# LuletterSoul/RP-Style-Transfer

Hardware: AMD Instinct MI355X
Metric: stylized images/sec at 512×512, 1/2/4/8 MI355X; % HBM roofline (higher is better)
Workload: dtype fp32

## Files before the change

rp-style-transfer_amd/csrc/rpst_wino4q.hip:

```cpp
#include "rpst_conv.h"

#include <type_traits>

#ifndef RPST_W4Q_DBG
#define RPST_W4Q_DBG 0
#endif

namespace rpst {
namespace {

template <int PAD>
__device__ __forceinline__ void q_mfma(floatx4& acc, float a, float b) {
  if constexpr (PAD)
    asm volatile("s_nop 1\n\tv_mfma_f32_16x16x4_f32 %0, %1, %2, %0" : "+v"(acc) : "v"(a), "v"(b));
  else
    asm volatile("v_mfma_f32_16x16x4_f32 %0, %1, %2, %0" : "+v"(acc) : "v"(a), "v"(b));
}
__device__ __forceinline__ unsigned q_lds_addr(const float* p) {
  return (unsigned)(uintptr_t)(const __attribute__((address_space(3))) float*)p;
}
template <int OFF>
__device__ __forceinline__ void q_dma16(__amdgpu_buffer_rsrc_t r, unsigned m0, unsigned voff,
                                        int soff) {
  asm volatile("s_mov_b32 m0, %0\n\ts_nop 0\n\tbuffer_load_dwordx4 %1, %2, %3 offen offset:%4 lds"
               :: "s"(m0), "v"(voff), "s"(r), "s"(soff), "i"(OFF) : "memory");
}
__device__ __forceinline__ void q_dma4(__amdgpu_buffer_rsrc_t r, unsigned m0, unsigned voff,
                                       int soff) {
  asm volatile("s_mov_b32 m0, %0\n\ts_nop 0\n\tbuffer_load_dword %1, %2, %3 offen lds"
               :: "s"(m0), "v"(voff), "s"(r), "s"(soff) : "memory");
}
__device__ __forceinline__ void q_lds_barrier() {
  asm volatile("s_waitcnt lgkmcnt(0)" ::: "memory");
  __builtin_amdgcn_s_barrier();
}

template <int H>
__device__ __forceinline__ void q_bt3(float d0, float d1, float d2, float d3, float d4, float d5,
                                      float& u0, float& u1, float& u2) {
  if constexpr (H == 0) {
    const float A = fmaf(-4.f, d2, d4), B = fmaf(-4.f, d1, d3);
    u0 = fmaf(4.f, d0, fmaf(-5.f, d2, d4));
    u1 = A + B;
    u2 = A - B;
  } else {
    const float C = d4 - d2, E = d3 - d1;
    u0 = fmaf(2.f, E, C);
    u1 = fmaf(-2.f, E, C);
    u2 = fmaf(4.f, d1, fmaf(-5.f, d3, d5));
  }
}

}

constexpr int kQCo = 64;
constexpr int kQTH = 8, kQTW = 64;
constexpr int kQXO = 4;
constexpr int kQPS = 72;
constexpr int kQCS = 768;
constexpr int kQWS = 9216;
constexpr int kQPAT = 4 * kQCS;
constexpr int kQNTH = 512;
constexpr int kQMaxCo = 512;
constexpr int kQWPI = 5;
constexpr int kQWide = 2, kQSlow = 6;
constexpr int kQDMA4 = 3, kQDMA = 12;
constexpr int kQRP = kQPS / 4;
constexpr int kQXS = 4 * 3 * 3 * 64 * 2;
constexpr int kQWG0 = 0;
constexpr int kQPG = 5;
constexpr int kQAhead = 3;
static_assert(10 * kQRP <= kQDMA4 * 64 && kQDMA4 * 256 <= kQCS, "16-B pieces in a channel");
static_assert(10 * kQPS <= kQDMA * 64 && kQDMA * 64 <= kQCS, "4-B pieces in a channel");
static_assert(2 * kQWide >= kQDMA4 && 2 * kQSlow >= kQDMA && 8 * kQWPI >= 36, "coverage");
static_assert(2 * kQXS <= kQWS, "the exchange fits a weight stage");
static_assert((2 * kQWS + 4 * kQPAT) * 4 + 1024 + kQSlow * kQNTH * 4 + 9 * kQMaxCo * 4 <= 163840,
              "LDS");

template <typename TW>
__global__ void wino4q_pack_kernel(const TW* __restrict__ w, float* __restrict__ pk, int Cout,
                                   int Cin, int K4, int64_t per, int64_t total, int64_t sco,
                                   int64_t sci, int64_t stap) {
  int64_t t = (int64_t)blockIdx.x * blockDim.x + threadIdx.x;
  if (t >= total) return;
  const int64_t img = t / per;
  pk += img * per;
  w += img * (int64_t)Cout * Cin * 9;
  t -= img * per;
  const int cb = (int)(t & 3);
  int64_t r = t >> 2;
  const int l = (int)(r & 63);
  r >>= 6;
  const int p = (int)(r % 9);
  r /= 9;
  const int q = (int)(r & 3);
  r >>= 2;
  const int ks = (int)(r % K4);
  const int ct = (int)(r / K4);
  const int i = 3 * (q >> 1) + p / 3, jj = 3 * (q & 1) + p % 3;
  const int co = ct * kQCo + cb * 16 + (l & 15);
  const int ci = ks * 4 + (l >> 4);
  float v = 0.f;
  if (co < Cout && ci < Cin) {
    const double G[6][3] = {{0.25, 0, 0},
                            {-1.0 / 6, -1.0 / 6, -1.0 / 6},
                            {-1.0 / 6, 1.0 / 6, -1.0 / 6},
                            {1.0 / 24, 1.0 / 12, 1.0 / 6},
                            {1.0 / 24, -1.0 / 12, 1.0 / 6},
                            {0, 0, 1}};
    const TW* g = w + co * sco + ci * sci;
    double acc = 0.0;
#pragma unroll
    for (int u = 0; u < 3; ++u)
#pragma unroll
      for (int s = 0; s < 3; ++s) acc += G[i][u] * (double)g[(u * 3 + s) * stap] * G[jj][s];
    v = (float)acc;
  }
  pk[t] = v;
}

size_t wino4q_packed_floats(int Cout, int Cin) {
  return (size_t)((Cout + kQCo - 1) / kQCo) * ((Cin + 3) / 4) * kQWS;
}

int wino4q_pack(const float* w, float* pk, int Cout, int Cin, hipStream_t st) {
  const int64_t t = (int64_t)wino4q_packed_floats(Cout, Cin);
  wino4q_pack_kernel<float><<<(unsigned)((t + 255) / 256), 256, 0, st>>>(
      w, pk, Cout, Cin, (Cin + 3) / 4, t, t, (int64_t)Cin * 9, 9, 1);
  return launch_status("wino4q_pack_kernel");
}

int wino4q_pack_mix(const double* wm, float* pk, int N, int Cout, int Cin, hipStream_t st) {
  const int64_t per = (int64_t)wino4q_packed_floats(Cout, Cin), tot = (int64_t)N * per;
  wino4q_pack_kernel<double><<<(unsigned)((tot + 255) / 256), 256, 0, st>>>(
      wm, pk, Cout, Cin, (Cin + 3) / 4, per, tot, Cin, 1, (int64_t)Cout * Cin);
  return launch_status("wino4q_pack_kernel(mix)");
}

__global__ void wino4q_fold_w_kernel(const float4* __restrict__ pk, float4* __restrict__ out,
                                     const float* __restrict__ aux, int N, int Cin, int K4,
                                     int64_t per4) {
  const int64_t t = (int64_t)blockIdx.x * blockDim.x + threadIdx.x;
  if (t >= (int64_t)N * per4) return;
  const int n = (int)(t / per4);
  const int64_t u = t - (int64_t)n * per4;
  const int l = (int)(u & 63);
  const int ks = (int)((u / (kQWS / 4)) % K4);
  const int ci = ks * 4 + (l >> 4);
  const int64_t nc = (int64_t)N * Cin, i = (int64_t)n * Cin + (ci < Cin ? ci : 0);
  const float sc = ci < Cin ? aux[3 * nc + i] / aux[2 * nc + i] : 0.f;
  const float4 v = pk[u];
  out[t] = make_float4(v.x * sc, v.y * sc, v.z * sc, v.w * sc);
}

int wino4q_fold_w(const float* pk, float* out, const float* aux, int N, int Cout, int Cin,
                  hipStream_t st) {
  const int64_t per4 = (int64_t)wino4q_packed_floats(Cout, Cin) / 4, n4 = (int64_t)N * per4;
  wino4q_fold_w_kernel<<<(unsigned)((n4 + 255) / 256), 256, 0, st>>>(
      reinterpret_cast<const float4*>(pk), reinterpret_cast<float4*>(out), aux, N, Cin,
      (Cin + 3) / 4, per4);
  return launch_status("wino4q_fold_w_kernel");
}

bool wino4q_applies(int Cin, int Cout, int in_op, const ConvMode& m) {
  const int min_cin = m.quarter == 2 ? 16 : 128;
  return m.quarter && m.precise != 2 && (in_op == RPST_IN_NONE || in_op == RPST_IN_UPSAMPLE2) &&
         Cout >= 64 && Cout <= kQMaxCo &&
         Cin >= min_cin && Cin % 16 == 0;
}

ConvTiling wino4q_tiling(ConvArgs& a) {
  a.Cout_pad = (a.Cout + kQCo - 1) / kQCo * kQCo;
  a.nchunks = (a.Cin + 3) / 4;
  a.tiles_x = (a.W + kQTW - 1) / kQTW;
  a.tiles_y = (a.H + kQTH - 1) / kQTH;
  a.co_tiles = a.Cout_pad / kQCo;
  a.stat_P = a.tiles_x * a.tiles_y * 2;
  a.cosplit = 1;
  return {(int64_t)a.tiles_x * a.tiles_y * a.N, kQNTH, 4, kQTH / 4, kQTW, true};
}

struct QEpi {
  int W, H, Cout, gy0, gx0, rows, n, sidx;
  bool vec, full, bst, edge, store, pool;
  float inv, slope;
  unsigned voff[4];
  float* out;
  float* oimg;
  unsigned obytes;
  const float* btab;
  float2* statp;
  int statP;
};

__device__ __forceinline__ QEpi q_epi_ctx(int wr, int tn) {
  const KArgs L = late_args();
  QEpi e;
  e.W = L->W;
  e.H = L->H;
  e.Cout = L->Cout;
  e.slope = L->relu == RPST_ACT_RELU ? 0.f : (L->relu == RPST_ACT_LRELU ? 0.2f : 1.f);
  int btx, bty;
  w4_tile((int)blockIdx.x / L->cosplit, L->tiles_x, L->tiles_y, btx, bty, e.n);
  const int bx0 = btx * kQTW;
  e.gy0 = bty * kQTH + 4 * wr;
  e.gx0 = bx0 + 4 * tn;
  e.vec = (e.W & 3) == 0 && e.gx0 + 3 < e.W;
  e.rows = max(0, min(4, e.H - e.gy0));
  const int cols = max(0, min(kQTW, e.W - bx0));
  e.inv = e.rows * cols > 0 ? __builtin_amdgcn_rcpf((float)(e.rows * cols)) : 0.f;
  e.full = e.rows == 4 && bx0 + kQTW <= e.W;
  e.edge = e.gy0 == 0 || e.gy0 + 4 >= e.H || bx0 == 0 || bx0 + kQTW >= e.W;
  e.out = L->out;
  const int64_t plane = (int64_t)e.H * e.W;
  e.pool = L->pool_out != 0;
  e.bst = !e.pool && (e.W & 3) == 0 && (int64_t)e.Cout * plane * 4 < (1LL << 31);
  e.oimg = e.out + (int64_t)e.n * e.Cout * plane;
  const bool keep = L->skip_from <= 0 || e.n < L->skip_from;
  e.obytes = keep ? (unsigned)(e.Cout * plane * 4) : 0u;
  e.store = keep;
#pragma unroll
  for (int yy = 0; yy < 4; ++yy)
    e.voff[yy] = (yy < e.rows && e.gx0 < e.W) ? (unsigned)(((e.gy0 + yy) * e.W + e.gx0) * 4)
                                             : 0x80000000u;
  e.btab = L->btab;
  e.statp = L->stat_part;
  e.statP = L->stat_P;
  e.sidx = (bty * L->tiles_x + btx) * 2 + wr;
  return e;
}

template <bool STATS, bool BTAB, bool RELU>
__device__ __forceinline__ void q_finish(const QEpi& e, int co, float (&Y)[16], int tn) {
  const int gy0 = e.gy0, gx0 = e.gx0, rows = e.rows, n = e.n;
  const bool cok = co < e.Cout;
  if constexpr (BTAB) {
    if (e.edge) {
      const float* bt = e.btab + (cok ? co : 0) * 9;
      float b9[9];
#pragma unroll
      for (int i = 0; i < 9; ++i) b9[i] = cok ? bt[i] : 0.f;
      const float b4 = b9[4];
#pragma unroll
      for (int i = 0; i < 9; ++i) b9[i] -= b4;
#pragma unroll
      for (int yy = 0; yy < 4; ++yy) {
        const int gy = gy0 + yy;
        const int rc = gy == 0 ? 0 : (gy >= e.H - 1 ? 2 : 1);
        const float l = rc == 0 ? b9[0] : (rc == 2 ? b9[6] : b9[3]);
        const float m = rc == 0 ? b9[1] : (rc == 2 ? b9[7] : b9[4]);
        const float r = rc == 0 ? b9[2] : (rc == 2 ? b9[8] : b9[5]);
#pragma unroll
        for (int xx = 0; xx < 4; ++xx) {
          const int gx = gx0 + xx;
          Y[yy * 4 + xx] += gx == 0 ? l : (gx >= e.W - 1 ? r : m);
        }
      }
    }
  }
#pragma unroll
  for (int i = 0; i < 16; ++i)
    Y[i] = __builtin_amdgcn_fmed3f(Y[i], RELU ? 0.f : e.slope * Y[i], __builtin_inff());
  float sum = 0.f;
  if constexpr (STATS) {
    if (e.full) {
#pragma unroll
      for (int i = 0; i < 16; ++i) sum += Y[i];
    } else {
#pragma unroll
      for (int yy = 0; yy < 4; ++yy)
#pragma unroll
        for (int xx = 0; xx < 4; ++xx) sum += (yy < rows && gx0 + xx < e.W) ? Y[yy * 4 + xx] : 0.f;
    }
  }
  if ((RPST_W4Q_DBG & 64) && e.statP > -7) {
  } else if (e.bst) {
    const auto ro = rsrc_or_zero(e.oimg, e.obytes, true);
    const unsigned cofs = cok ? (unsigned)co * (unsigned)(e.H * e.W) * 4u : 0x7fffffffu;
#pragma unroll
    for (int yy = 0; yy < 4; ++yy) {
      const floatx4 v = {Y[yy * 4], Y[yy * 4 + 1], Y[yy * 4 + 2], Y[yy * 4 + 3]};
      __builtin_amdgcn_raw_buffer_store_b128(__builtin_bit_cast(u32x4, v), ro,
                                             (int)(e.voff[yy] + cofs), 0, 0);
    }
  } else if (e.pool) {
    if (cok && e.store) {
      const int Ho = (e.H + 1) >> 1, Wo = (e.W + 1) >> 1;
      float* o = e.out + (((int64_t)n * e.Cout + co) * Ho + (gy0 >> 1)) * Wo + (gx0 >> 1);
#pragma unroll
      for (int py = 0; py < 2; ++py) {
        if (2 * py >= rows) continue;
        const bool y1 = 2 * py + 1 < rows;
        float pv[2];
#pragma unroll
        for (int px = 0; px < 2; ++px) {
          const bool x1 = gx0 + 2 * px + 1 < e.W;
          const float* t = Y + (2 * py) * 4 + 2 * px;
          float v = t[0];
          if (x1) v = fmaxf(v, t[1]);
          if (y1) v = fmaxf(v, t[4]);
          if (x1 && y1) v = fmaxf(v, t[5]);
          pv[px] = v;
        }
        if (gx0 + 3 < e.W && (Wo & 1) == 0) {
          *reinterpret_cast<float2*>(o + py * Wo) = make_float2(pv[0], pv[1]);
        } else {
          if (gx0 < e.W) o[py * Wo] = pv[0];
          if (gx0 + 2 < e.W) o[py * Wo + 1] = pv[1];
        }
      }
    }
  } else if (cok && e.store) {
    float* o = e.out + (((int64_t)n * e.Cout + co) * e.H + gy0) * e.W + gx0;
#pragma unroll
    for (int yy = 0; yy < 4; ++yy) {
      if (yy < rows) {
        if (e.vec) {
          *reinterpret_cast<float4*>(o + yy * e.W) =
              make_float4(Y[yy * 4], Y[yy * 4 + 1], Y[yy * 4 + 2], Y[yy * 4 + 3]);
        } else {
#pragma unroll
          for (int xx = 0; xx < 4; ++xx)
            if (gx0 + xx < e.W) o[yy * e.W + xx] = Y[yy * 4 + xx];
        }
      }
    }
  }
  if constexpr (STATS) {
    sum = row16_sum(sum);
    const float mean = sum * e.inv;
    float m2 = 0.f;
    if (e.full) {
#pragma unroll
      for (int i = 0; i < 16; ++i) m2 = fmaf(Y[i] - mean, Y[i] - mean, m2);
    } else {
#pragma unroll
      for (int yy = 0; yy < 4; ++yy)
#pragma unroll
        for (int xx = 0; xx < 4; ++xx) {
          const float dv = Y[yy * 4 + xx] - mean;
          m2 += (yy < rows && gx0 + xx < e.W) ? dv * dv : 0.f;
        }
    }
    m2 = row16_sum(m2);
    if (tn == 0 && cok)
      e.statp[((int64_t)n * e.statP + e.sidx) * e.Cout + co] = make_float2(mean, m2);
  }
}

template <int INOP, bool STATS, bool BTAB, bool RELU>
__global__ __launch_bounds__(kQNTH, 1) void wino4q_mfma_kernel(ConvArgs a) {
  __shared__ __attribute__((aligned(16))) float ws0[kQWS];
  __shared__ __attribute__((aligned(16))) float ws1[kQWS];
  __shared__ __attribute__((aligned(16))) float ps0[kQPAT];
  __shared__ __attribute__((aligned(16))) float ps1[kQPAT];
  __shared__ __attribute__((aligned(16))) float ps2[kQPAT];
  __shared__ __attribute__((aligned(16))) float ps3[kQPAT];
  __shared__ __attribute__((aligned(16))) float dummy[256];
  __shared__ unsigned poffs[kQSlow][kQNTH];
  __shared__ float btl[BTAB ? 9 * kQMaxCo : kQMaxCo];

  const int wave = __builtin_amdgcn_readfirstlane((int)threadIdx.x >> 6);
  const int lane = threadIdx.x & 63;
  const int k = lane >> 4, tn = lane & 15, wr = wave >> 2;

  int bid = (int)blockIdx.x;
  const int cog = bid % a.cosplit;
  bid /= a.cosplit;
  const int nct = a.co_tiles / a.cosplit, ct0 = cog * nct;
  int tx, ty, n;
  w4_tile(bid, a.tiles_x, a.tiles_y, tx, ty, n);
  const int K4 = a.nchunks, G = nct * K4;
  const int y0 = ty * kQTH, x0 = tx * kQTW;

  {
    const int nb = BTAB ? 9 * a.Cout : a.Cout;
    const float* src = BTAB ? a.btab + (int64_t)n * nb : a.bias;
    for (int i = threadIdx.x; i < nb; i += kQNTH) btl[i] = src ? src[i] : 0.f;
  }
  constexpr bool up = INOP == RPST_IN_UPSAMPLE2;
  const unsigned in_plane = up ? (unsigned)(a.Hs * a.Ws) : (unsigned)(a.H * a.W);
  const unsigned oob = a.Cin * in_plane * 4u;
  const float* in_img = conv_in_img(a, n, (int64_t)a.Cin * in_plane);
  const unsigned wbytes = (unsigned)(nct * K4 * kQWS) * 4u;
  const float* w_img = a.wpk + (int64_t)n * a.wstride + (int64_t)ct0 * K4 * kQWS;

  const int hf = wave & 1;
  const bool zp = a.pad == RPST_PAD_ZERO;
  const int rs = up ? a.Ws : a.W;
  const bool w4a = (a.W & 3) == 0;
  const bool wide = !up && ((x0 >= 1 && x0 + kQTW < a.W) || (w4a && x0 + kQTW <= a.W));
  const bool fixL = wide && w4a && !zp && x0 == 0;
  const bool fixR = wide && w4a && !zp && x0 + kQTW == a.W;
  unsigned poff[kQSlow];
  const int tid = threadIdx.x;
  if (wide) {
#pragma unroll
    for (int i = 0; i < kQWide; ++i) {
      const int p = kQWide * hf + i;
      const int f = 64 * p + lane, row = min(f / kQRP, 9), j = f - (f / kQRP) * kQRP;
      int y = y0 - 1 + row;
      const int xs = x0 - kQXO + 4 * j;
      const bool okx = !w4a || (xs >= 0 && xs + 3 < a.W);
      const bool ok = p < kQDMA4 && f < 10 * kQRP && resolve_bf(y, a.H, zp) && okx;
      poff[i] = ok ? ((unsigned)(y * rs) + (unsigned)xs) * 4u : oob;
    }
#pragma unroll
    for (int i = kQWide; i < kQSlow; ++i) poff[i] = oob;
  } else {
#pragma unroll
    for (int i = 0; i < kQSlow; ++i) {
      const int p = kQSlow * hf + i;
      const int f = 64 * p + lane;
      const int row = min(f / kQPS, 9), col = f - (f / kQPS) * kQPS;
      int y = y0 - 1 + row, x = x0 - kQXO + col;
      const bool oky = resolve_bf(y, a.H, zp), okx = resolve_bf(x, a.W, zp);
      const bool ok = p < kQDMA && col >= kQXO - 1 && col < kQXO + 1 + kQTW &&
                      f < 10 * kQPS && oky && okx;
      poff[i] = ok ? ((unsigned)((up ? y >> 1 : y) * rs) + (unsigned)(up ? x >> 1 : x)) * 4u : oob;
    }
  }
#pragma unroll
  for (int i = 0; i < kQSlow; ++i) poffs[i][tid] = poff[i];

  constexpr int DBG = RPST_W4Q_DBG;
  const int wl = wave * 4096;
  const bool real4 = wave < 4;
  const int w4 = 32768 + wave * 1024;
  const unsigned dummy_a = q_lds_addr(dummy);
  int wso = wl;
  auto issue_w = [&](bool live, unsigned stg, auto Ic) {
    constexpr int I = decltype(Ic)::value;
    if (DBG & 2) return;
    if constexpr (I < 4) {
      q_dma16<1024 * I>(rsrc_or_zero(w_img, wbytes, live), stg + wl, lane * 16, wso);
    } else {
      q_dma16<0>(rsrc_or_zero(w_img, wbytes, live && real4), real4 ? stg + w4 : dummy_a,
                 lane * 16, wso + (w4 - wl));
    }
  };
  const unsigned pstep = 4u * in_plane * 4u;
  const int pbase = (int)((unsigned)(wave >> 1) * in_plane * 4u);
  const bool h1 = (wave & 1) != 0;
  const int pl = (wave >> 1) * (kQCS * 4) + (h1 ? (wide ? 2048 : kQSlow * 256) : 0);
  int pso = pbase;
  auto issue_p = [&](auto WIDEc, bool live, unsigned stg) {
    constexpr bool WIDE = decltype(WIDEc)::value;
    if (DBG & 1) return;
    const auto r = rsrc_or_zero(in_img, oob, live);
    const unsigned xs = stg + launder(pl);
    if constexpr (WIDE) {
      q_dma16<0>(r, xs, poffs[0][tid], pso);
      q_dma16<0>(r, h1 ? dummy_a : xs + 1024, poffs[1][tid], pso);
    } else {
#pragma unroll
      for (int i = 0; i < kQSlow; ++i) q_dma4(r, xs + 256 * i, poffs[i][tid], pso);
    }
    pso += (int)pstep;
  };
  const bool bst_all = !a.pool_out && (a.W & 3) == 0 &&
                       (int64_t)a.Cout * a.H * a.W * 4 < (1LL << 31);
  bool post_epi = false;
  auto wait_ring = [&](bool first) {
    if (DBG & 128) return;
    if (first && post_epi && bst_all) {
      if (wide) asm volatile("s_waitcnt vmcnt(18)" ::: "memory");
      else asm volatile("s_waitcnt vmcnt(22)" ::: "memory");
    } else if (wide) {
      asm volatile("s_waitcnt vmcnt(2)" ::: "memory");
    } else {
      asm volatile("s_waitcnt vmcnt(6)" ::: "memory");
    }
    if (first) post_epi = false;
  };

  auto fix_halo = [&](float* stg) {
    if ((wave == 0 && fixL) || (wave == 1 && fixR)) {
      int l = lane;
      asm volatile("" : "+v"(l));
      if (l < 40) {
        const int ch = l / 10, row = l - 10 * ch;
        float* rp = stg + ch * kQCS + row * kQPS;
        if (wave == 0) rp[kQXO - 1] = rp[kQXO + 1];
        else rp[kQXO + kQTW] = rp[kQXO + kQTW - 2];
      }
    }
  };
  auto prologue = [&](auto WIDEc) {
    issue_p(WIDEc, true, q_lds_addr(ps0));
    issue_p(WIDEc, true, q_lds_addr(ps1));
    issue_w(true, q_lds_addr(ws0), std::integral_constant<int, 0>{});
    issue_w(true, q_lds_addr(ws0), std::integral_constant<int, 1>{});
    issue_w(true, q_lds_addr(ws0), std::integral_constant<int, 2>{});
    issue_w(true, q_lds_addr(ws0), std::integral_constant<int, 3>{});
    issue_w(true, q_lds_addr(ws0), std::integral_constant<int, 4>{});
    issue_p(WIDEc, true, q_lds_addr(ps2));
    issue_p(WIDEc, true, q_lds_addr(ps3));
  };
  if (wide) prologue(std::true_type{});
  else prologue(std::false_type{});
  wait_ring(false);
  q_lds_barrier();
  if (fixL || fixR) {
    fix_halo(ps0);
    fix_halo(ps1);
    q_lds_barrier();
  }

  auto body = [&](auto Qc) {
    constexpr int Q = decltype(Qc)::value, QR = Q >> 1, QC = Q & 1;
    floatx4 acc[9][4];
#pragma unroll
    for (int p = 0; p < 9; ++p)
#pragma unroll
      for (int cb = 0; cb < 4; ++cb) acc[p][cb] = floatx4{0.f, 0.f, 0.f, 0.f};
    const int roff = k * kQCS + (4 * wr + QR) * kQPS + 4 * tn;
    auto read_row = [&](const float* stg, int rr, float (&d)[8]) {
      const float* rp = stg + roff + rr * kQPS;
      floatx4 u = *reinterpret_cast<const floatx4*>(rp + 4);
      const float e = QC ? rp[8] : rp[3];
      asm("" : "+v"(u));
      d[0] = QC ? 0.f : e; d[1] = u[0]; d[2] = u[1]; d[3] = u[2]; d[4] = u[3];
      d[5] = QC ? e : 0.f; d[6] = 0.f; d[7] = 0.f;
    };
    auto col_pass = [&](const float (&d)[8], float (&u)[3]) {
      if (DBG & 8) {
        u[0] = d[0]; u[1] = d[1]; u[2] = d[2];
        return;
      }
      q_bt3<QC>(d[0], d[1], d[2], d[3], d[4], d[5], u[0], u[1], u[2]);
    };
    auto row_pass = [&](const float (&u)[5][3], int j, float (&v)[9]) {
      if (DBG & 8) {
        v[j] = u[0][j]; v[3 + j] = u[2][j]; v[6 + j] = u[4][j];
        return;
      }
      if constexpr (QR == 0)
        q_bt3<0>(u[0][j], u[1][j], u[2][j], u[3][j], u[4][j], 0.f, v[j], v[3 + j], v[6 + j]);
      else
        q_bt3<1>(0.f, u[0][j], u[1][j], u[2][j], u[3][j], u[4][j], v[j], v[3 + j], v[6 + j]);
    };
    float V[9];
    {
      float u[5][3];
#pragma unroll
      for (int rr = 0; rr < 5; ++rr) {
        float d[8];
        read_row(ps0, rr, d);
        col_pass(d, u[rr]);
      }
#pragma unroll
      for (int j = 0; j < 3; ++j) row_pass(u, j, V);
    }

    const int woff = Q * 9 * 256 + lane * 4;
    int x = 0;
    auto step = [&](float* wsx, float* psn, float* wsn, float* psx, float* pfx, int ks,
                    bool first) {
      wait_ring(first);
      const bool wlive = x + 1 < G, plive = x + 4 < G;
      wso += kQWS * 4;
      if (first && ks + 4 == K4) pso = pbase;
      const unsigned wsn_a = q_lds_addr(wsn), psx_a = q_lds_addr(psx);
      if (DBG & 16) asm volatile("s_waitcnt lgkmcnt(0)" ::: "memory");
      else q_lds_barrier();
      constexpr int ord[9] = {0, 3, 6, 1, 4, 7, 2, 5, 8};
      constexpr int kA = kQAhead;
      float4 w4[9];
#pragma unroll
      for (int q = 0; q < kA; ++q)
        w4[ord[q]] = *reinterpret_cast<const float4*>(wsx + woff + ord[q] * 256);
      float d[8];
      read_row(psn, 0, d);
      float u[5][3];
#pragma unroll
      for (int q = 0; q < 9; ++q) {
        const int p = ord[q];
        if (q + kA < 9)
          w4[ord[q + kA]] = *reinterpret_cast<const float4*>(wsx + woff + ord[q + kA] * 256);
        q_mfma<1>(acc[p][0], w4[p].x, V[p]);
        q_mfma<0>(acc[p][1], w4[p].y, V[p]);
        q_mfma<0>(acc[p][2], w4[p].z, V[p]);
        q_mfma<0>(acc[p][3], w4[p].w, V[p]);
        if (q == kQWG0) issue_w(wlive, wsn_a, std::integral_constant<int, 0>{});
        if (q == kQWG0 + 1) issue_w(wlive, wsn_a, std::integral_constant<int, 1>{});
        if (q == kQWG0 + 2) issue_w(wlive, wsn_a, std::integral_constant<int, 2>{});
        if (q == kQWG0 + 3) issue_w(wlive, wsn_a, std::integral_constant<int, 3>{});
        if (q == kQWG0 + 4) issue_w(wlive, wsn_a, std::integral_constant<int, 4>{});
        if (q == kQPG) {
          if (wide) issue_p(std::true_type{}, plive, psx_a);
          else issue_p(std::false_type{}, plive, psx_a);
        }
        if (q < 5) {
          col_pass(d, u[q]);
          if (q + 1 < 5) read_row(psn, q + 1, d);
        }
        if (q == 5 || q == 6 || q == 8) row_pass(u, q == 8 ? 2 : q - 5, V);
        if (q == 7) fix_halo(pfx);
      }
      ++x;
    };

    auto epilogue = [&](int ctile) {
      if (DBG & 32) {
        float t = 0.f;
#pragma unroll
        for (int p = 0; p < 9; ++p)
#pragma unroll
          for (int cb = 0; cb < 4; ++cb) t += acc[p][cb][0];
        if (t == 1.2345f) late_args()->out[threadIdx.x] = t;
#pragma unroll
        for (int p = 0; p < 9; ++p)
#pragma unroll
          for (int cb = 0; cb < 4; ++cb) acc[p][cb] = floatx4{0.f, 0.f, 0.f, 0.f};
        return;
      }
      q_lds_barrier();
      asm volatile("s_nop 7\n\ts_nop 4" : "+v"(acc[0][0]), "+v"(acc[0][1]), "+v"(acc[0][2]),
                   "+v"(acc[0][3]), "+v"(acc[1][0]), "+v"(acc[1][1]), "+v"(acc[1][2]),
                   "+v"(acc[1][3]), "+v"(acc[2][0]), "+v"(acc[2][1]), "+v"(acc[2][2]),
                   "+v"(acc[2][3]), "+v"(acc[3][0]), "+v"(acc[3][1]), "+v"(acc[3][2]),
                   "+v"(acc[3][3]), "+v"(acc[4][0]), "+v"(acc[4][1]));
      asm volatile("" : "+v"(acc[4][2]), "+v"(acc[4][3]), "+v"(acc[5][0]), "+v"(acc[5][1]),
                   "+v"(acc[5][2]), "+v"(acc[5][3]), "+v"(acc[6][0]), "+v"(acc[6][1]),
                   "+v"(acc[6][2]), "+v"(acc[6][3]), "+v"(acc[7][0]), "+v"(acc[7][1]),
                   "+v"(acc[7][2]), "+v"(acc[7][3]), "+v"(acc[8][0]), "+v"(acc[8][1]),
                   "+v"(acc[8][2]), "+v"(acc[8][3]));
      const int co0 = ctile * kQCo + 16 * Q + 4 * k;
#pragma unroll
      for (int rp = 0; rp < 2; ++rp) {
        float P[2][6][4];
#pragma unroll
        for (int pt = 0; pt < 3; ++pt) {
          float* xb = ws1 + wr * kQXS;
#pragma unroll
          for (int dq = 0; dq < 4; ++dq) {
            if (dq == Q || (DBG & 4)) continue;
            const int slot = (Q - dq - 1) & 3;
#pragma unroll
            for (int j = 0; j < 3; ++j)
              *reinterpret_cast<float2*>(xb + (((dq * 3 + slot) * 3 + j) * 64 + lane) * 2) =
                  make_float2(acc[3 * pt + j][dq][2 * rp], acc[3 * pt + j][dq][2 * rp + 1]);
          }
          if (!(DBG & 4)) q_lds_barrier();
          float m[2][2][6];
#pragma unroll
          for (int s = 0; s < 4; ++s) {
#pragma unroll
            for (int j = 0; j < 3; ++j) {
              float2 v;
              if (s == Q || (DBG & 4)) {
                const int src = (DBG & 4) ? s : Q;
                v = make_float2(acc[3 * pt + j][src][2 * rp], acc[3 * pt + j][src][2 * rp + 1]);
              } else {
                v = *reinterpret_cast<const float2*>(
                    xb + (((Q * 3 + ((s - Q - 1) & 3)) * 3 + j) * 64 + lane) * 2);
              }
              m[0][s >> 1][3 * (s & 1) + j] = v.x;
              m[1][s >> 1][3 * (s & 1) + j] = v.y;
            }
          }
#pragma unroll
          for (int e2 = 0; e2 < 2; ++e2) {
            at6(m[e2][0], P[e2][pt]);
            at6(m[e2][1], P[e2][3 + pt]);
          }
          if (!(DBG & 4) && (rp == 0 || pt < 2)) q_lds_barrier();
        }
#pragma unroll
        for (int e2 = 0; e2 < 2; ++e2) {
          const int r = 2 * rp + e2;
          QEpi e = q_epi_ctx(wr, tn);
          e.btab = btl;
          float bias = 0.f;
          {
            const int co = co0 + r;
            if (co < e.Cout) bias = BTAB ? btl[co * 9 + 4] : btl[co];
          }
#pragma unroll
          for (int x = 0; x < 4; ++x) P[e2][1][x] += bias;
          float Y[16];
#pragma unroll
          for (int x = 0; x < 4; ++x) {
            float c6[6], y[4];
#pragma unroll
            for (int I = 0; I < 6; ++I) c6[I] = P[e2][I][x];
            at6(c6, y);
#pragma unroll
            for (int yy = 0; yy < 4; ++yy) Y[yy * 4 + x] = y[yy];
          }
          q_finish<STATS, BTAB, RELU>(e, co0 + r, Y, tn);
        }
      }
#pragma unroll
      for (int p = 0; p < 9; ++p)
#pragma unroll
        for (int cb = 0; cb < 4; ++cb) acc[p][cb] = floatx4{0.f, 0.f, 0.f, 0.f};
    };

    int ks = 0, ct = ct0;
    for (int g = 0; g < G; g += 4) {
      step(ws0, ps1, ws1, ps0, ps2, ks, true);
      step(ws1, ps2, ws0, ps1, ps3, ks + 1, false);
      step(ws0, ps3, ws1, ps2, ps0, ks + 2, false);
      step(ws1, ps0, ws0, ps3, ps1, ks + 3, false);
      ks += 4;
      if (ks == K4) {
        epilogue(ct);
        post_epi = true;
        ks = 0;
        ++ct;
      }
    }
  };
  switch (wave & 3) {
    case 0: body(std::integral_constant<int, 0>{}); break;
    case 1: body(std::integral_constant<int, 1>{}); break;
    case 2: body(std::integral_constant<int, 2>{}); break;
    default: body(std::integral_constant<int, 3>{}); break;
  }
  asm volatile("s_waitcnt vmcnt(0)" ::: "memory");
}

int wino4q_launch(ConvArgs& a, int in_op, hipStream_t st) {
  RPST_REQUIRE(in_op == RPST_IN_NONE || in_op == RPST_IN_UPSAMPLE2,
               "conv2d: winograd4 (quarter) does not support in_op %d", in_op);
  const ConvTiling t = wino4q_tiling(a);
  RPST_REQUIRE((int64_t)a.co_tiles * a.nchunks * kQWS * 4 < (1LL << 31),
               "conv2d: winograd4 weight image exceeds 2 GiB");
  RPST_REQUIRE(t.blocks <= 0x7fffffffLL, "conv2d: grid too large");
  const unsigned nb = (unsigned)t.blocks;
  const bool stats = a.stat_part != nullptr, btab = a.btab != nullptr;
  RPST_REQUIRE(!btab || in_op == RPST_IN_NONE, "conv2d: winograd4 bias table with a loader op");
  RPST_REQUIRE(!(stats && btab), "conv2d: winograd4 folded bias with statistics");
#define RPST_W4Q_GO(OP, S, B)                                                  \
  do {                                                                         \
    if (a.relu == RPST_ACT_RELU)                                               \
      wino4q_mfma_kernel<OP, S, B, true><<<nb, kQNTH, 0, st>>>(a);             \
    else                                                                       \
      wino4q_mfma_kernel<OP, S, B, false><<<nb, kQNTH, 0, st>>>(a);            \
  } while (0)
  if (in_op == RPST_IN_UPSAMPLE2) {
    if (stats) RPST_W4Q_GO(RPST_IN_UPSAMPLE2, true, false);
    else RPST_W4Q_GO(RPST_IN_UPSAMPLE2, false, false);
  } else {
    if (stats) RPST_W4Q_GO(RPST_IN_NONE, true, false);
    else if (btab) RPST_W4Q_GO(RPST_IN_NONE, false, true);
    else RPST_W4Q_GO(RPST_IN_NONE, false, false);
  }
#undef RPST_W4Q_GO
  return launch_status("wino4q_mfma_kernel");
}

}
```

Before: 570.9.

## Add all-wide Winograd kernel variant and stats-only epilogue for skipped images

Adds a WIDE_ALL template specialization, chosen when the width is a multiple of the tile width. It removes the runtime wide/slow branching, shrinks the per-thread offset tables and fixes the vmcnt waits at compile time. It also adds a stats-only epilogue path: for images at or beyond skip_from, output stores and their address setup are skipped while statistics are still computed, and post_epi tracking is adjusted so the next wait_ring does not wait on stores that were never issued. The cost is more kernel instantiations and extra divergence in the epilogue logic.

```diff
diff --git a/rp-style-transfer_amd/csrc/rpst_wino4q.hip b/rp-style-transfer_amd/csrc/rpst_wino4q.hip
--- a/rp-style-transfer_amd/csrc/rpst_wino4q.hip
+++ b/rp-style-transfer_amd/csrc/rpst_wino4q.hip
@@ -193,6 +193,7 @@
   int statP;
 };
 
+template <bool STORE>
 __device__ __forceinline__ QEpi q_epi_ctx(int wr, int tn) {
   const KArgs L = late_args();
   QEpi e;
@@ -211,18 +212,26 @@
   e.inv = e.rows * cols > 0 ? __builtin_amdgcn_rcpf((float)(e.rows * cols)) : 0.f;
   e.full = e.rows == 4 && bx0 + kQTW <= e.W;
   e.edge = e.gy0 == 0 || e.gy0 + 4 >= e.H || bx0 == 0 || bx0 + kQTW >= e.W;
-  e.out = L->out;
-  const int64_t plane = (int64_t)e.H * e.W;
-  e.pool = L->pool_out != 0;
-  e.bst = !e.pool && (e.W & 3) == 0 && (int64_t)e.Cout * plane * 4 < (1LL << 31);
-  e.oimg = e.out + (int64_t)e.n * e.Cout * plane;
-  const bool keep = L->skip_from <= 0 || e.n < L->skip_from;
-  e.obytes = keep ? (unsigned)(e.Cout * plane * 4) : 0u;
-  e.store = keep;
-#pragma unroll
-  for (int yy = 0; yy < 4; ++yy)
-    e.voff[yy] = (yy < e.rows && e.gx0 < e.W) ? (unsigned)(((e.gy0 + yy) * e.W + e.gx0) * 4)
-                                             : 0x80000000u;
+  if constexpr (STORE) {
+    e.out = L->out;
+    const int64_t plane = (int64_t)e.H * e.W;
+    e.pool = L->pool_out != 0;
+    e.bst = !e.pool && (e.W & 3) == 0 && (int64_t)e.Cout * plane * 4 < (1LL << 31);
+    e.oimg = e.out + (int64_t)e.n * e.Cout * plane;
+    const bool keep = L->skip_from <= 0 || e.n < L->skip_from;
+    e.obytes = keep ? (unsigned)(e.Cout * plane * 4) : 0u;
+    e.store = keep;
+#pragma unroll
+    for (int yy = 0; yy < 4; ++yy)
+      e.voff[yy] = (yy < e.rows && e.gx0 < e.W) ? (unsigned)(((e.gy0 + yy) * e.W + e.gx0) * 4)
+                                               : 0x80000000u;
+  } else {
+    e.out = e.oimg = nullptr;
+    e.obytes = 0u;
+    e.pool = e.bst = e.store = false;
+#pragma unroll
+    for (int yy = 0; yy < 4; ++yy) e.voff[yy] = 0x80000000u;
+  }
   e.btab = L->btab;
   e.statp = L->stat_part;
   e.statP = L->stat_P;
@@ -230,7 +239,7 @@
   return e;
 }
 
-template <bool STATS, bool BTAB, bool RELU>
+template <bool STATS, bool BTAB, bool RELU, bool STORE = true>
 __device__ __forceinline__ void q_finish(const QEpi& e, int co, float (&Y)[16], int tn) {
   const int gy0 = e.gy0, gx0 = e.gx0, rows = e.rows, n = e.n;
   const bool cok = co < e.Cout;
@@ -273,7 +282,9 @@
         for (int xx = 0; xx < 4; ++xx) sum += (yy < rows && gx0 + xx < e.W) ? Y[yy * 4 + xx] : 0.f;
     }
   }
-  if ((RPST_W4Q_DBG & 64) && e.statP > -7) {
+  if constexpr (!STORE) {
+  } else if ((RPST_W4Q_DBG & 64) && e.statP > -7) {
+  } else if ((RPST_W4Q_DBG & 256) && !e.store) {
   } else if (e.bst) {
     const auto ro = rsrc_or_zero(e.oimg, e.obytes, true);
     const unsigned cofs = cok ? (unsigned)co * (unsigned)(e.H * e.W) * 4u : 0x7fffffffu;
@@ -348,8 +359,9 @@
   }
 }
 
-template <int INOP, bool STATS, bool BTAB, bool RELU>
+template <int INOP, bool STATS, bool BTAB, bool RELU, bool WIDE_ALL = false>
 __global__ __launch_bounds__(kQNTH, 1) void wino4q_mfma_kernel(ConvArgs a) {
+  static_assert(!WIDE_ALL || INOP == RPST_IN_NONE, "an all-wide launch has no loader operator");
   __shared__ __attribute__((aligned(16))) float ws0[kQWS];
   __shared__ __attribute__((aligned(16))) float ws1[kQWS];
   __shared__ __attribute__((aligned(16))) float ps0[kQPAT];
@@ -357,7 +369,8 @@
   __shared__ __attribute__((aligned(16))) float ps2[kQPAT];
   __shared__ __attribute__((aligned(16))) float ps3[kQPAT];
   __shared__ __attribute__((aligned(16))) float dummy[256];
-  __shared__ unsigned poffs[kQSlow][kQNTH];
+  constexpr int NPO = WIDE_ALL ? kQWide : kQSlow;
+  __shared__ unsigned poffs[NPO][kQNTH];
   __shared__ float btl[BTAB ? 9 * kQMaxCo : kQMaxCo];
 
   const int wave = __builtin_amdgcn_readfirstlane((int)threadIdx.x >> 6);
@@ -388,11 +401,12 @@
   const int hf = wave & 1;
   const bool zp = a.pad == RPST_PAD_ZERO;
   const int rs = up ? a.Ws : a.W;
-  const bool w4a = (a.W & 3) == 0;
-  const bool wide = !up && ((x0 >= 1 && x0 + kQTW < a.W) || (w4a && x0 + kQTW <= a.W));
+  const bool w4a = WIDE_ALL || (a.W & 3) == 0;
+  const bool wide = WIDE_ALL || (RPST_W4Q_DBG & 512) ||
+                    (!up && ((x0 >= 1 && x0 + kQTW < a.W) || (w4a && x0 + kQTW <= a.W)));
   const bool fixL = wide && w4a && !zp && x0 == 0;
   const bool fixR = wide && w4a && !zp && x0 + kQTW == a.W;
-  unsigned poff[kQSlow];
+  unsigned poff[NPO];
   const int tid = threadIdx.x;
   if (wide) {
 #pragma unroll
@@ -406,8 +420,8 @@
       poff[i] = ok ? ((unsigned)(y * rs) + (unsigned)xs) * 4u : oob;
     }
 #pragma unroll
-    for (int i = kQWide; i < kQSlow; ++i) poff[i] = oob;
-  } else {
+    for (int i = kQWide; i < NPO; ++i) poff[i] = oob;
+  } else if constexpr (!WIDE_ALL) {
 #pragma unroll
     for (int i = 0; i < kQSlow; ++i) {
       const int p = kQSlow * hf + i;
@@ -421,7 +435,7 @@
     }
   }
 #pragma unroll
-  for (int i = 0; i < kQSlow; ++i) poffs[i][tid] = poff[i];
+  for (int i = 0; i < NPO; ++i) poffs[i][tid] = poff[i];
 
   constexpr int DBG = RPST_W4Q_DBG;
   const int wl = wave * 4096;
@@ -458,14 +472,30 @@
     }
     pso += (int)pstep;
   };
+  auto issue_pb = [&](bool live, unsigned stg) {
+    if constexpr (WIDE_ALL) {
+      issue_p(std::true_type{}, live, stg);
+    } else {
+      if (wide) issue_p(std::true_type{}, live, stg);
+      else issue_p(std::false_type{}, live, stg);
+    }
+  };
   const bool bst_all = !a.pool_out && (a.W & 3) == 0 &&
                        (int64_t)a.Cout * a.H * a.W * 4 < (1LL << 31);
+  __shared__ int sonly;
+  if (STATS && threadIdx.x == 0) sonly = !(DBG & 256) && a.skip_from > 0 && n >= a.skip_from;
   bool post_epi = false;
   auto wait_ring = [&](bool first) {
     if (DBG & 128) return;
     if (first && post_epi && bst_all) {
-      if (wide) asm volatile("s_waitcnt vmcnt(18)" ::: "memory");
-      else asm volatile("s_waitcnt vmcnt(22)" ::: "memory");
+      if constexpr (WIDE_ALL) {
+        asm volatile("s_waitcnt vmcnt(18)" ::: "memory");
+      } else {
+        if (wide) asm volatile("s_waitcnt vmcnt(18)" ::: "memory");
+        else asm volatile("s_waitcnt vmcnt(22)" ::: "memory");
+      }
+    } else if constexpr (WIDE_ALL) {
+      asm volatile("s_waitcnt vmcnt(2)" ::: "memory");
     } else if (wide) {
       asm volatile("s_waitcnt vmcnt(2)" ::: "memory");
     } else {
@@ -497,8 +527,12 @@
     issue_p(WIDEc, true, q_lds_addr(ps2));
     issue_p(WIDEc, true, q_lds_addr(ps3));
   };
-  if (wide) prologue(std::true_type{});
-  else prologue(std::false_type{});
+  if constexpr (WIDE_ALL) {
+    prologue(std::true_type{});
+  } else {
+    if (wide) prologue(std::true_type{});
+    else prologue(std::false_type{});
+  }
   wait_ring(false);
   q_lds_barrier();
   if (fixL || fixR) {
@@ -514,7 +548,9 @@
     for (int p = 0; p < 9; ++p)
 #pragma unroll
       for (int cb = 0; cb < 4; ++cb) acc[p][cb] = floatx4{0.f, 0.f, 0.f, 0.f};
-    const int roff = k * kQCS + (4 * wr + QR) * kQPS + 4 * tn;
+    int kb = k;
+    if constexpr (STATS) asm volatile("" : "+v"(kb));
+    const int roff = kb * kQCS + (4 * wr + QR) * kQPS + 4 * tn;
     auto read_row = [&](const float* stg, int rr, float (&d)[8]) {
       const float* rp = stg + roff + rr * kQPS;
       floatx4 u = *reinterpret_cast<const floatx4*>(rp + 4);
@@ -587,10 +623,7 @@
         if (q == kQWG0 + 2) issue_w(wlive, wsn_a, std::integral_constant<int, 2>{});
         if (q == kQWG0 + 3) issue_w(wlive, wsn_a, std::integral_constant<int, 3>{});
         if (q == kQWG0 + 4) issue_w(wlive, wsn_a, std::integral_constant<int, 4>{});
-        if (q == kQPG) {
-          if (wide) issue_p(std::true_type{}, plive, psx_a);
-          else issue_p(std::false_type{}, plive, psx_a);
-        }
+        if (q == kQPG) issue_pb(plive, psx_a);
         if (q < 5) {
           col_pass(d, u[q]);
           if (q + 1 < 5) read_row(psn, q + 1, d);
@@ -613,9 +646,12 @@
         for (int p = 0; p < 9; ++p)
 #pragma unroll
           for (int cb = 0; cb < 4; ++cb) acc[p][cb] = floatx4{0.f, 0.f, 0.f, 0.f};
+        post_epi = true;
         return;
       }
       q_lds_barrier();
+      bool stats_only = false;
+      if constexpr (STATS) stats_only = __builtin_amdgcn_readfirstlane(sonly) != 0;
       asm volatile("s_nop 7\n\ts_nop 4" : "+v"(acc[0][0]), "+v"(acc[0][1]), "+v"(acc[0][2]),
                    "+v"(acc[0][3]), "+v"(acc[1][0]), "+v"(acc[1][1]), "+v"(acc[1][2]),
                    "+v"(acc[1][3]), "+v"(acc[2][0]), "+v"(acc[2][1]), "+v"(acc[2][2]),
@@ -670,12 +706,10 @@
 #pragma unroll
         for (int e2 = 0; e2 < 2; ++e2) {
           const int r = 2 * rp + e2;
-          QEpi e = q_epi_ctx(wr, tn);
-          e.btab = btl;
           float bias = 0.f;
           {
             const int co = co0 + r;
-            if (co < e.Cout) bias = BTAB ? btl[co * 9 + 4] : btl[co];
+            if (co < late_args()->Cout) bias = BTAB ? btl[co * 9 + 4] : btl[co];
           }
 #pragma unroll
           for (int x = 0; x < 4; ++x) P[e2][1][x] += bias;
@@ -689,13 +723,22 @@
 #pragma unroll
             for (int yy = 0; yy < 4; ++yy) Y[yy * 4 + x] = y[yy];
           }
-          q_finish<STATS, BTAB, RELU>(e, co0 + r, Y, tn);
+          if (STATS && stats_only) {
+            QEpi e = q_epi_ctx<false>(wr, tn);
+            e.btab = btl;
+            q_finish<STATS, BTAB, RELU, false>(e, co0 + r, Y, tn);
+          } else {
+            QEpi e = q_epi_ctx<true>(wr, tn);
+            e.btab = btl;
+            q_finish<STATS, BTAB, RELU, true>(e, co0 + r, Y, tn);
+          }
         }
       }
 #pragma unroll
       for (int p = 0; p < 9; ++p)
 #pragma unroll
         for (int cb = 0; cb < 4; ++cb) acc[p][cb] = floatx4{0.f, 0.f, 0.f, 0.f};
+      post_epi = !stats_only;
     };
 
     int ks = 0, ct = ct0;
@@ -707,7 +750,6 @@
       ks += 4;
       if (ks == K4) {
         epilogue(ct);
-        post_epi = true;
         ks = 0;
         ++ct;
       }
@@ -733,22 +775,29 @@
   const bool stats = a.stat_part != nullptr, btab = a.btab != nullptr;
   RPST_REQUIRE(!btab || in_op == RPST_IN_NONE, "conv2d: winograd4 bias table with a loader op");
   RPST_REQUIRE(!(stats && btab), "conv2d: winograd4 folded bias with statistics");
-#define RPST_W4Q_GO(OP, S, B)                                                  \
+  const bool all_wide = in_op == RPST_IN_NONE && (a.W & 3) == 0 && a.W % kQTW == 0;
+#define RPST_W4Q_GO2(OP, S, B, WA)                                             \
   do {                                                                         \
     if (a.relu == RPST_ACT_RELU)                                               \
-      wino4q_mfma_kernel<OP, S, B, true><<<nb, kQNTH, 0, st>>>(a);             \
+      wino4q_mfma_kernel<OP, S, B, true, WA><<<nb, kQNTH, 0, st>>>(a);         \
     else                                                                       \
-      wino4q_mfma_kernel<OP, S, B, false><<<nb, kQNTH, 0, st>>>(a);            \
+      wino4q_mfma_kernel<OP, S, B, false, WA><<<nb, kQNTH, 0, st>>>(a);        \
+  } while (0)
+#define RPST_W4Q_GO(S, B)                                                      \
+  do {                                                                         \
+    if (all_wide) RPST_W4Q_GO2(RPST_IN_NONE, S, B, true);                      \
+    else RPST_W4Q_GO2(RPST_IN_NONE, S, B, false);                              \
   } while (0)
   if (in_op == RPST_IN_UPSAMPLE2) {
-    if (stats) RPST_W4Q_GO(RPST_IN_UPSAMPLE2, true, false);
-    else RPST_W4Q_GO(RPST_IN_UPSAMPLE2, false, false);
+    if (stats) RPST_W4Q_GO2(RPST_IN_UPSAMPLE2, true, false, false);
+    else RPST_W4Q_GO2(RPST_IN_UPSAMPLE2, false, false, false);
   } else {
-    if (stats) RPST_W4Q_GO(RPST_IN_NONE, true, false);
-    else if (btab) RPST_W4Q_GO(RPST_IN_NONE, false, true);
-    else RPST_W4Q_GO(RPST_IN_NONE, false, false);
+    if (stats) RPST_W4Q_GO(true, false);
+    else if (btab) RPST_W4Q_GO(false, true);
+    else RPST_W4Q_GO(false, false);
   }
 #undef RPST_W4Q_GO
+#undef RPST_W4Q_GO2
   return launch_status("wino4q_mfma_kernel");
 }
 
```

Result: no change. 575.4 (median of 6 runs) (+0.8%).
